# mlaaks/coherent-rtlsdr

Hardware: AMD Instinct MI355X
Metric: aligned IQ blocks/s (1024 ch x 8192) (higher is better)
Workload: dtype f32

## Files before the change

coherent-rtlsdr_amd/csrc/crsdr.hip:

```cpp
#include "../../include/crsdr.h"
#include "kernels.hpp"
#include "doa.hpp"

#include <hip/hip_runtime.h>

#include <cctype>
#include <cmath>
#include <cstdarg>
#include <cstdio>
#include <cstdlib>
#include <cstring>
#include <mutex>
#include <new>
#include <string>
#include <vector>
#include <sched.h>

using namespace crsdr;

static thread_local char g_err[512] = "";

static int fail(int code, const char *fmt, ...)
{
    va_list ap;
// ... 130 lines not shown
static int make_twiddles14(float2 **d_twA, float2 **d_twB)
{
    std::vector<float2> a(5 * 512), b(5 * 16);
    for (int j = 0; j < 5; ++j) {
        for (int t = 0; t < 512; ++t) {
            double ang = 2.0 * M_PI * (double)(t << j) / 16384.0;
            a[j * 512 + t] = make_float2((float)std::cos(ang), (float)(-std::sin(ang)));
        }
        for (int n = 0; n < 16; ++n) {
            double ang = 2.0 * M_PI * (double)(n << j) / 512.0;
            b[j * 16 + n] = make_float2((float)std::cos(ang), (float)(-std::sin(ang)));
        }
    }
    HIP_TRY(hipMalloc((void **)d_twA, sizeof(float2) * a.size()));
    HIP_TRY(hipMalloc((void **)d_twB, sizeof(float2) * b.size()));
    HIP_TRY(hipMemcpy(*d_twA, a.data(), sizeof(float2) * a.size(), hipMemcpyHostToDevice));
    HIP_TRY(hipMemcpy(*d_twB, b.data(), sizeof(float2) * b.size(), hipMemcpyHostToDevice));
    return CRSDR_OK;
}

static int make_twiddle_table(double n, size_t count, size_t step, float2 **d)
{
    std::vector<float2> h(count);
    for (size_t k = 0; k < count; ++k) {
        double a = 2.0 * M_PI * (double)(k * step) / n;
        h[k] = make_float2((float)std::cos(a), (float)(-std::sin(a)));
    }
    HIP_TRY(hipMalloc((void **)d, sizeof(float2) * count));
    HIP_TRY(hipMemcpy(*d, h.data(), sizeof(float2) * count, hipMemcpyHostToDevice));
    return CRSDR_OK;
}

constexpr int kMinLog2 = 4, kMaxLog2 = 14, kMaxLog2Plan = 22;

template <int LOG2N>
static constexpr size_t fft_lds_bytes() { return sizeof(float2) * ((size_t)1 << LOG2N) + 256; }

struct SpinSwitch {
    int value, dflt;
    long from;
    int at(long launch) const { return launch >= from ? value : dflt; }
};
static SpinSwitch spin_switch(const char *e, int dflt)
{
    const char *at = e ? strchr(e, '@') : nullptr;
    return {e ? atoi(e) : dflt, dflt, at ? atol(at + 1) : 0L};
}
struct Switches {
    char k1_variant;
    SpinSwitch qspin;
    SpinSwitch refspin;
    int k2_spin;
    bool long_q;
};
static const Switches &sw()
{
    static const Switches s = [] {
        const char *v = getenv("CRSDR_K1_VARIANT"), *lq = getenv("CRSDR_LONG_Q");
        const char c = v ? v[0] : 'a';
        return Switches{(c == 'p' || c == 'q') ? c : 'a', spin_switch(getenv("CRSDR_K1_QSPIN"), x14p::kQSpinLimit),
                        spin_switch(getenv("CRSDR_K1_REFSPIN"), kRefWaitBudget), spin_switch(getenv("CRSDR_K2_SPIN"), kFusedSpinLimit).value,
                        !lq || atoi(lq) != 0};
    }();
    return s;
}

static int device_cus()
{
    static const int cus = [] {
        int dev = 0, n = 0;
        if (hipGetDevice(&dev) != hipSuccess || hipDeviceGetAttribute(&n, hipDeviceAttributeMultiprocessorCount, dev) != hipSuccess || n < 1) n = 256;
        return n;
    }();
    return cus;
}
static char k1_pick(int rows_all, bool allow_q)
{
    char variant = sw().k1_variant;
    if (variant == 'a') variant = rows_all >= 12 * device_cus() ? 'q' : 'p';
    if (variant == 'q' && !allow_q) variant = 'p';
    return variant;
}

template <typename Kernel, typename... Args>
static hipError_t launch_lds(Kernel kern, dim3 grid, dim3 block, size_t lds, hipStream_t s, const Args &...args)
{
    const hipError_t e = hipFuncSetAttribute((const void *)kern, hipFuncAttributeMaxDynamicSharedMemorySize, (int)lds);
    if (e != hipSuccess) return e;
    hipLaunchKernelGGL(kern, grid, block, lds, s, args...);
    return hipGetLastError();
}

template <int LOG2N>
static hipError_t launch_ref_spectrum(hipStream_t s, int nblocks, const int8_t *rows, size_t block_stride, const float2 *tw,
                                      float2 *refspec, uint32_t xor80)
{
    return launch_lds(k_ref_spectrum<LOG2N>, dim3(nblocks), dim3(FftGeom<LOG2N>::THREADS), fft_lds_bytes<LOG2N>(), s, rows, block_stride, tw,
                      refspec, xor80);
}

template <int LOG2N>
static hipError_t launch_xcorr_lag(hipStream_t s, const XcorrArgs &a, int row_count, const float2 *tw)
{
    return launch_lds(k_xcorr_lag<LOG2N>, dim3(row_count, a.nblocks), dim3(FftGeom<LOG2N>::THREADS), fft_lds_bytes<LOG2N>(), s, a, tw);
}

static hipError_t launch_ref_spectrum14(hipStream_t s, int nblocks, const int8_t *rows, size_t block_stride, const float2 *twA,
                                        const float2 *twB, float2 *refspec, uint32_t xor80)
{
    return launch_lds(x14p::k_ref_spectrum14p, dim3(nblocks), dim3(x14::THREADS), x14::LDS_BYTES, s, rows, block_stride,
                      reinterpret_cast<const c2 *>(twA), reinterpret_cast<const c2 *>(twB), (float4 *)refspec, xor80);
}

static hipError_t launch_xcorr_lag14(hipStream_t s, char variant, const XcorrArgs &a, int row_count, const float2 *twA, const float2 *twB,
                                     int *waitflag, unsigned int *work, unsigned int *work_base)
{
    const int items = row_count * a.nblocks + (a.fold ? a.nblocks : 0);
    if (variant != 'q')
        return launch_lds(x14p::k_xcorr_lag14p, dim3((unsigned)items), dim3(x14::THREADS), x14::LDS_BYTES, s, a, twA, twB, row_count);
    static long launches = 0;
    const int qspin = sw().qspin.at(launches++);
    const hipError_t e = launch_lds(x14p::k_xcorr_lag14q, dim3((unsigned)std::max(1, std::min(device_cus(), (items + 1) / 2))), dim3(2 * x14p::QG),
                                    x14p::LDSQ_BYTES, s, a, twA, twB, row_count, waitflag, work, *work_base, qspin);
    if (e == hipSuccess) *work_base += (unsigned)items;
    return e;
}

template <int LOG2N, int DIR>
static hipError_t launch_op_fft(hipStream_t s, int howmany, float2 *out, const float2 *in, const float2 *tw)
{
    return launch_lds(k_op_fft<LOG2N, DIR>, dim3(howmany), dim3(FftGeom<LOG2N>::THREADS), fft_lds_bytes<LOG2N>(), s, out, in, tw);
}

#define CRSDR_DISPATCH_N1(l2, CALL)                                                     \
    [&]() -> hipError_t {                                                               \
        switch (l2) {                                                                   \
        case 1: { constexpr int LG = 1; return CALL; }                                  \
        case 2: { constexpr int LG = 2; return CALL; }                                  \
        case 3: { constexpr int LG = 3; return CALL; }                                  \
        case 4: { constexpr int LG = 4; return CALL; }                                  \
        case 5: { constexpr int LG = 5; return CALL; }                                  \
        case 6: { constexpr int LG = 6; return CALL; }                                  \
        case 7: { constexpr int LG = 7; return CALL; }                                  \
        case 8: { constexpr int LG = 8; return CALL; }                                  \
        default: return hipErrorInvalidValue;                                           \
        }                                                                               \
    }()

static int lb_grid(int nwork, bool stage_c = false)
{
    const int per_cu = stage_c ? 0 : 2;
#ifdef CRSDR_LB_EXPERIMENT
    static const int dbg_set = [] { const char *e = getenv("CRSDR_LB_DBG"); int v = e ? atoi(e) : 0; (void)hipMemcpyToSymbol(HIP_SYMBOL(lb::lb_dbg), &v, sizeof(v)); return v; }();
    (void)dbg_set;
#endif
    return per_cu > 0 ? std::max(1, std::min(nwork, per_cu * device_cus())) : nwork;
}
template <int LOG2N1, bool IS_REF>
static hipError_t launch_long_fwd_cols(hipStream_t s, int nrows_launch, const int8_t *rows, int row_begin, uint32_t xor80,
                                       const lb::LongTw &tw, float2 *Y)
{
    const int nwork = lb::ntiles(LOG2N1) * nrows_launch;
    return launch_lds(lb::k_long_fwd_cols<LOG2N1, IS_REF>, dim3((unsigned)lb_grid(nwork)), dim3(lb::THREADS), lb::LDS_BYTES, s, rows, row_begin,
                      xor80, tw, Y, nwork);
}
static hipError_t launch_long_rows_q(hipStream_t s, int n1, int nrows_launch, float2 *Y, const float2 *twA, const float2 *twB, float2 *refspec,
                                     int *waitflag, const x14p::RampArgs *ramp = nullptr, float2 *Yout = nullptr)
{
    const int items = n1 * nrows_launch;
    const int grid = std::max(1, std::min(device_cus(), (items + 1) / 2));
    const int nq = (!ramp && n1 % 8 == 0 && grid % 8 == 0) ? 8 : 1;
    static long launches = 0;
    const int qspin = sw().qspin.at(launches++);
    return launch_lds(ramp ? x14p::k_rows14_cf32q<true> : x14p::k_rows14_cf32q<false>, dim3((unsigned)grid), dim3(2 * x14p::QG), x14p::LDSQ_BYTES, s,
                      reinterpret_cast<c2 *>(Y), reinterpret_cast<const c2 *>(twA), reinterpret_cast<const c2 *>(twB), (const float4 *)refspec, n1,
// ... 323 lines not shown
    if (mem_kind == CRSDR_MEM_HOST) HIP_TRY(hipMemcpy(pm, d_p, pb, hipMemcpyDeviceToHost));
    else HIP_TRY(hipDeviceSynchronize());
    return CRSDR_OK;
}

constexpr int kStageSlots = 4;
constexpr unsigned kWaitTwoRow = 1u, kWaitTwoLine = 2u, kWaitFoldRef = 4u;
constexpr int kMaxBatch = 64;

struct crsdr_plan {
    int nrows = 0, B = 0, L = 0, log2n = 0, mode = 0, device = 0, row_begin = 1, row_count = 0, max_batch = 1;
    size_t packet_bytes = 0, matrix_off = 0, packet_stride = 0, own_packet_stride = 0;
    hipStream_t own_stream = nullptr, stream = nullptr, aux = nullptr;
    hipEvent_t ev_fork = nullptr, ev_ref[2] = {nullptr, nullptr}, ev_k1done[2] = {nullptr, nullptr};
    hipStream_t cs = nullptr;
    hipEvent_t ev_copydone[4] = {nullptr, nullptr, nullptr, nullptr};
    unsigned long copy_head = 0, copy_tail = 0;
    int *h_k1flag = nullptr;
    bool copy_pending = false;
    hipEvent_t ev_k2done[2] = {nullptr, nullptr};
    int obuf = 0;
    hipEvent_t ev_start = nullptr, ev_stop = nullptr;
    bool k1done_valid[2] = {false, false};
    bool fold_last[2] = {false, false};
    int slot = 0;
    float2 *d_tw = nullptr, *d_twA = nullptr, *d_twB = nullptr, *d_refspec[2] = {nullptr, nullptr};
    int8_t *d_rows = nullptr;
    uint8_t *d_packet_alloc = nullptr;
    int8_t *d_packet_own = nullptr, *d_packet = nullptr;
    int8_t *d_slab = nullptr;
    size_t slab_stride = 0, tail_offset = 0;
    int hdr_first = 0, hdr_count = 0;
    uint32_t *d_readcnt = nullptr;
    uint8_t *d_mask = nullptr;
    int32_t *d_lag = nullptr, *d_lag_state = nullptr;
    float *d_mag = nullptr, *d_frac = nullptr, *d_mag_state = nullptr, *d_frac_state = nullptr;
    float2 *d_phasor = nullptr, *d_phase_state[2] = {nullptr, nullptr};
    long long *d_corr = nullptr;
    int chain_slot = 0;
    int chain_armed[2] = {0, 0};
    unsigned int *d_sync = nullptr;
    unsigned int q_work_base = 0;
    bool k1_used = false;
    unsigned k1_waits = 0;
    uint8_t *d_state = nullptr, *d_state_snap = nullptr;
    size_t state_bytes = 0;
    bool q_disabled = false;
    static constexpr int kSnaps = 8;
    struct Snap { unsigned long idx; int phase_cur; } snaps[kSnaps] = {};
    int snap_head = 0, snap_cnt = 0;
    unsigned long submit_idx = 0;
    unsigned long copy_idx[4] = {0, 0, 0, 0};
    bool fused_k2 = true;
    bool fold = true;
    unsigned int *d_refflag = nullptr, refgen = 0;
    int phase_cur = 0;
    int last_nblocks = 0;
    bool longblock = false;
    int log2n1 = 0;
    float2 *d_wc = nullptr, *d_wf = nullptr, *d_tw1 = nullptr, *d_Y = nullptr, *d_Yref = nullptr;
    lb::LongPartial *d_part = nullptr;
    int long_chunk = 1 << 30;
    bool frac_apply = false, frac_override_on = false;
    float frac_gain = 1.0f;
    float *d_frac_override = nullptr;
    uint32_t *d_k2tab = nullptr;
    bool frac_generic = false;
    float2 *d_Z = nullptr;
    float4 *d_rowspec = nullptr;
    uint32_t *h_readcnt = nullptr;
    uint8_t *h_mask = nullptr;
    hipEvent_t ev_stage[kStageSlots] = {};
    bool stage_valid[kStageSlots] = {};
    int stage_slot = 0;
    bool submitted = false;
    int prof_slots = 0;
    uint32_t prof_mask = 0;
    long prof_count = 0;
    std::vector<hipEvent_t> prof_ev;
    std::vector<unsigned char> prof_has;
};

constexpr int kProfKernels = 4;

static hipEvent_t *prof_pair(crsdr_plan *p, int which)
{
    if (!p->prof_slots || !(p->prof_mask & (1u << which))) return nullptr;
    const int slot = (int)(p->prof_count % p->prof_slots);
    p->prof_has[(size_t)slot * kProfKernels + which] = 1;
    return &p->prof_ev[((size_t)slot * kProfKernels + which) * 2];
}

static int plan_init_state(crsdr_plan *p)
{
    const size_t n = (size_t)p->nrows, T = (size_t)p->max_batch;
    std::vector<float2> ph(n, make_float2(1.0f, 0.0f));
    ph[0] = make_float2(0.0f, 0.0f);
    for (int i = 0; i < 2; ++i) HIP_TRY(hipMemcpy(p->d_phase_state[i], ph.data(), sizeof(float2) * n, hipMemcpyHostToDevice));
    for (size_t t = 0; t < T; ++t) HIP_TRY(hipMemcpy(p->d_phasor + t * n, ph.data(), sizeof(float2) * n, hipMemcpyHostToDevice));
    HIP_TRY(hipMemset(p->d_lag, 0, sizeof(int32_t) * n * T * 2));
    HIP_TRY(hipMemset(p->d_mag, 0, sizeof(float) * n * T * 2));
    HIP_TRY(hipMemset(p->d_frac, 0, sizeof(float) * n * T * 2));
    HIP_TRY(hipMemset(p->d_lag_state, 0, sizeof(int32_t) * n));
    HIP_TRY(hipMemset(p->d_mag_state, 0, sizeof(float) * n));
    HIP_TRY(hipMemset(p->d_frac_state, 0, sizeof(float) * n));
    HIP_TRY(hipMemset(p->d_corr, 0xFF, sizeof(long long) * 4 * n * T));
    p->chain_armed[0] = p->chain_armed[1] = (int)T;
// ... 38 lines not shown
{
    HIP_TRY(hipSetDevice(p->device));
    HIP_TRY(hipStreamCreateWithFlags(&p->own_stream, hipStreamNonBlocking));
    HIP_TRY(hipStreamCreateWithFlags(&p->aux, hipStreamNonBlocking));
    HIP_TRY(hipStreamCreateWithFlags(&p->cs, hipStreamNonBlocking));
    for (auto &e : p->ev_copydone) HIP_TRY(hipEventCreateWithFlags(&e, hipEventDisableTiming));
    HIP_TRY(hipHostMalloc((void **)&p->h_k1flag, 4 * sizeof(int), hipHostMallocDefault));
    memset(p->h_k1flag, 0, 4 * sizeof(int));
    p->stream = p->own_stream;
    hipEvent_t *evs[] = {&p->ev_fork, &p->ev_ref[0], &p->ev_ref[1], &p->ev_k1done[0], &p->ev_k1done[1], &p->ev_k2done[0], &p->ev_k2done[1]};
    for (auto e : evs) HIP_TRY(hipEventCreateWithFlags(e, hipEventDisableTiming));
    for (int i = 0; i < kStageSlots; ++i) HIP_TRY(hipEventCreateWithFlags(&p->ev_stage[i], hipEventDisableTiming));
    HIP_TRY(hipEventCreate(&p->ev_start));
    HIP_TRY(hipEventCreate(&p->ev_stop));
    { int rc = make_twiddles(p->longblock ? lb::N2 : p->B, &p->d_tw); if (rc) return rc; }
    if (p->log2n == 14 || p->longblock) { int rc = make_twiddles14(&p->d_twA, &p->d_twB); if (rc) return rc; }
    if (p->longblock) {
        const size_t Bz = (size_t)p->B, n1 = Bz >> lb::LOG2N2;
        int rc;
        if ((rc = make_twiddle_table((double)Bz, Bz >> lb::FBITS, (size_t)1 << lb::FBITS, &p->d_wc))) return rc;
        if ((rc = make_twiddle_table((double)Bz, (size_t)1 << lb::FBITS, 1, &p->d_wf))) return rc;
        if ((rc = make_twiddle_table((double)n1, n1, 1, &p->d_tw1))) return rc;
        HIP_TRY(hipMalloc((void **)&p->d_Y, sizeof(float2) * Bz * (size_t)p->row_count));
        HIP_TRY(hipMalloc((void **)&p->d_Yref, sizeof(float2) * Bz));
        {
            const char *e = getenv("CRSDR_LONG_CHUNK_MB");
            const long mb = e ? atol(e) : 400;
            if (mb > 0) p->long_chunk = (int)std::max<size_t>(1, ((size_t)mb << 20) / (sizeof(float2) * Bz));
        }
        HIP_TRY(hipMalloc((void **)&p->d_part, sizeof(lb::LongPartial) * (size_t)lb::ntiles(p->log2n1) * (size_t)p->row_count));
    }
    const size_t n = (size_t)p->nrows, T = (size_t)p->max_batch;
    const size_t rowbytes = n * (size_t)p->B;
    for (int i = 0; i < 2; ++i) HIP_TRY(hipMalloc((void **)&p->d_refspec[i], sizeof(float2) * (size_t)p->B * T));
    HIP_TRY(hipMalloc((void **)&p->d_rows, rowbytes * T));
    const size_t pad = (256 - (p->matrix_off % 256)) % 256;
    p->own_packet_stride = (p->packet_bytes + 255) / 256 * 256;
    p->packet_stride = p->own_packet_stride;
    HIP_TRY(hipMalloc((void **)&p->d_packet_alloc, pad + p->own_packet_stride * T + 256));
    HIP_TRY(hipMemset(p->d_packet_alloc, 0, pad + p->own_packet_stride * T + 256));
    p->d_packet_own = reinterpret_cast<int8_t *>(p->d_packet_alloc + pad);
    p->d_packet = p->d_packet_own;
    HIP_TRY(hipMalloc((void **)&p->d_readcnt, sizeof(uint32_t) * n * T));
    HIP_TRY(hipMalloc((void **)&p->d_mask, n));
    HIP_TRY(hipMalloc((void **)&p->d_lag, sizeof(int32_t) * n * T * 2));
    HIP_TRY(hipMalloc((void **)&p->d_mag, sizeof(float) * n * T * 2));
    HIP_TRY(hipMalloc((void **)&p->d_frac, sizeof(float) * n * T * 2));
    HIP_TRY(hipMalloc((void **)&p->d_phasor, sizeof(float2) * n * T));
    HIP_TRY(hipMalloc((void **)&p->d_corr, sizeof(long long) * 4 * n * T));
    HIP_TRY(hipMalloc((void **)&p->d_sync, 64));
    HIP_TRY(hipMemset(p->d_sync, 0, 64));
    HIP_TRY(hipMalloc((void **)&p->d_refflag, sizeof(unsigned int) * T));
    HIP_TRY(hipMemset(p->d_refflag, 0, sizeof(unsigned int) * T));
    { const char *e = getenv("CRSDR_K1_FOLD"); if (e) p->fold = atoi(e) != 0; }
    { const char *e = getenv("CRSDR_K2_FUSED"); if (e) p->fused_k2 = atoi(e) != 0; }
    { const char *e = getenv("CRSDR_FRAC_GENERIC"); if (e) p->frac_generic = atoi(e) != 0; }
    {
        const size_t n8 = (n + 1) / 2 * 2;
        p->state_bytes = n8 * (3 * 4 + 2 * 8);
        HIP_TRY(hipMalloc((void **)&p->d_state, p->state_bytes));
        HIP_TRY(hipMalloc((void **)&p->d_state_snap, p->state_bytes * crsdr_plan::kSnaps));
        p->d_phase_state[0] = reinterpret_cast<float2 *>(p->d_state);
        p->d_phase_state[1] = p->d_phase_state[0] + n8;
        p->d_lag_state = reinterpret_cast<int32_t *>(p->d_phase_state[1] + n8);
        p->d_mag_state = reinterpret_cast<float *>(p->d_lag_state + n8);
        p->d_frac_state = p->d_mag_state + n8;
    }
    HIP_TRY(hipHostMalloc((void **)&p->h_readcnt, sizeof(uint32_t) * n * T * kStageSlots, hipHostMallocDefault));
    HIP_TRY(hipHostMalloc((void **)&p->h_mask, n * kStageSlots, hipHostMallocDefault));
    if (p->longblock || p->log2n == 14) { int rc = make_k2tab(p); if (rc) return rc; }
    HIP_TRY(hipMalloc((void **)&p->d_frac_override, sizeof(float) * (size_t)p->nrows));
    HIP_TRY(hipMemset(p->d_frac_override, 0, sizeof(float) * (size_t)p->nrows));
    return plan_init_state(p);
}

static void plan_free(crsdr_plan *p)
{
    if (!p) return;
    (void)hipSetDevice(p->device);
    if (p->own_stream) (void)hipStreamSynchronize(p->own_stream);
    if (p->aux) (void)hipStreamSynchronize(p->aux);
    if (p->cs) { (void)hipStreamSynchronize(p->cs); (void)hipStreamDestroy(p->cs); }
    for (auto e : p->ev_copydone) if (e) (void)hipEventDestroy(e);
    void *bufs[] = {p->d_Z, p->d_rowspec, p->d_frac_override, p->d_k2tab, p->d_wc, p->d_wf, p->d_tw1, p->d_Y, p->d_Yref, p->d_part, p->d_tw, p->d_twA, p->d_twB, p->d_refspec[0], p->d_refspec[1], p->d_rows, p->d_packet_alloc, p->d_readcnt,
                    p->d_mask, p->d_lag, p->d_mag, p->d_frac, p->d_phasor, p->d_corr, p->d_sync, p->d_state, p->d_state_snap, p->d_refflag};
    for (void *b : bufs) if (b) (void)hipFree(b);
    if (p->h_k1flag) (void)hipHostFree(p->h_k1flag);
    if (p->h_readcnt) (void)hipHostFree(p->h_readcnt);
    if (p->h_mask) (void)hipHostFree(p->h_mask);
    hipEvent_t evs[] = {p->ev_fork, p->ev_ref[0], p->ev_ref[1], p->ev_k1done[0], p->ev_k1done[1], p->ev_k2done[0], p->ev_k2done[1], p->ev_start, p->ev_stop};
    for (hipEvent_t e : evs) if (e) (void)hipEventDestroy(e);
    for (int i = 0; i < kStageSlots; ++i) if (p->ev_stage[i]) (void)hipEventDestroy(p->ev_stage[i]);
    for (hipEvent_t e : p->prof_ev) if (e) (void)hipEventDestroy(e);
    if (p->own_stream) (void)hipStreamDestroy(p->own_stream);
    if (p->aux) (void)hipStreamDestroy(p->aux);
    delete p;
}

extern "C" int crsdr_plan_create(crsdr_plan **plan, const crsdr_plan_desc *desc)
{
    if (!plan || !desc) return fail(CRSDR_EINVAL, "plan_create: NULL argument");
    *plan = nullptr;
    const int l2 = ilog2_exact(desc->blocksize);
    if (desc->nrows < 2) return fail(CRSDR_EINVAL, "plan_create: nrows = %d (need the ref row and >= 1 signal row)", desc->nrows);
    if (l2 < kMinLog2 || l2 > kMaxLog2Plan)
        return fail(CRSDR_EINVAL, "plan_create: blocksize = %d unsupported (power of two in [16, 4194304])", desc->blocksize);
    if (desc->mode != CRSDR_MODE_FAITHFUL && desc->mode != CRSDR_MODE_DIGITAL)
// ... 145 lines not shown
                return fail(CRSDR_EINVAL, "plan_set_frac_apply: frac_override[%d] = %g (need |D| <= 64 samples; larger delays belong in the integer lag)", r, (double)frac_override[r]);
    HIP_TRY(hipSetDevice(p->device));
    if (frac_override) {
        int rc = crsdr_plan_sync(p);
        if (rc) return rc;
        HIP_TRY(hipMemcpy(p->d_frac_override, frac_override, sizeof(float) * (size_t)p->nrows, hipMemcpyHostToDevice));
    }
    if (!p->longblock) {
        p->frac_apply = true; p->frac_gain = gain; p->frac_override_on = frac_override != nullptr;
        return CRSDR_OK;
    }
    if (!p->d_rowspec) HIP_TRY(hipMalloc((void **)&p->d_rowspec, sizeof(float4) * 8192 * (size_t)p->row_count));
    if (enable == 2 && p->d_Z) {
        int rc = crsdr_plan_sync(p);
        if (rc) return rc;
        (void)hipFree(p->d_Z);
        p->d_Z = nullptr;
    }
    if (enable == 1 && !p->d_Z && hipMalloc((void **)&p->d_Z, sizeof(float2) * (size_t)p->B * (size_t)p->row_count) != hipSuccess) {
        p->d_Z = nullptr;
        (void)hipGetLastError();
    }
    p->frac_apply = true; p->frac_gain = gain; p->frac_override_on = frac_override != nullptr;
    return CRSDR_OK;
}

static hipError_t take_snapshot(crsdr_plan *p, hipStream_t s)
{
    if (p->snap_cnt == crsdr_plan::kSnaps) return hipSuccess;
    if (p->snap_cnt && p->snaps[(p->snap_head + p->snap_cnt - 1) % crsdr_plan::kSnaps].idx == p->submit_idx) return hipSuccess;
    const int pos = (p->snap_head + p->snap_cnt) % crsdr_plan::kSnaps;
    const hipError_t e = hipMemcpyAsync(p->d_state_snap + (size_t)pos * p->state_bytes, p->d_state, p->state_bytes, hipMemcpyDeviceToDevice, s);
    if (e != hipSuccess) return e;
    p->snaps[pos].idx = p->submit_idx;
    p->snaps[pos].phase_cur = p->phase_cur;
    p->snap_cnt++;
    return hipSuccess;
}
static void retire_snapshots(crsdr_plan *p, unsigned long k)
{
    while (p->snap_cnt >= 2 && p->snaps[(p->snap_head + 1) % crsdr_plan::kSnaps].idx <= k + 1) { p->snap_head = (p->snap_head + 1) % crsdr_plan::kSnaps; p->snap_cnt--; }
    if (p->snap_cnt == 1 && p->snaps[p->snap_head].idx <= k && p->submit_idx == k + 1) p->snap_cnt = 0;
}

struct Batch {
    int nblocks;
    const int8_t *d_in;
    size_t d_stride;
    bool input_ready;
    uint32_t xor80;
    const uint32_t *d_readcnt;
    const uint8_t *d_mask;
    bool any_lag;
    int32_t *o_lag;
    float *o_mag, *o_frac;
    AlignArgs aa;
    bool vec16;
    int chunks;
    bool fused;
    bool kept_fwd;
    bool corr_zeroed;
};

static int stage_inputs(crsdr_plan *p, Batch &b, const void *rows, int mem_kind, size_t block_stride, const uint32_t *readcnt,
                        const uint8_t *lag_mask, uint32_t flags)
{
    hipStream_t S = p->stream;
    const size_t B = (size_t)p->B, n = (size_t)p->nrows, T = (size_t)b.nblocks;
    b.d_in = (const int8_t *)rows;
    b.d_stride = block_stride;
    b.input_ready = (flags & CRSDR_INPUT_READY) && mem_kind == CRSDR_MEM_DEVICE;
    b.xor80 = (flags & CRSDR_OFFSET_BINARY) ? 0x80808080u : 0u;
    if (mem_kind == CRSDR_MEM_HOST) {
        for (size_t t = 0; t < T; ++t) {
            const int8_t *src = (const int8_t *)rows + t * block_stride;
            int8_t *dst = p->d_rows + t * n * B;
            HIP_TRY(hipMemcpyAsync(dst, src, B, hipMemcpyHostToDevice, S));
            HIP_TRY(hipMemcpyAsync(dst + B * (size_t)p->row_begin, src + B * (size_t)p->row_begin, B * (size_t)p->row_count,
                                   hipMemcpyHostToDevice, S));
        }
        b.d_in = p->d_rows;
        b.d_stride = n * B;
    }
    b.any_lag = !(flags & CRSDR_NO_LAG);
    if (readcnt || lag_mask) {
        const int ss = p->stage_slot;
        p->stage_slot = (ss + 1) % kStageSlots;
        if (p->stage_valid[ss]) HIP_TRY(hipEventSynchronize(p->ev_stage[ss]));
        if (readcnt) {
            uint32_t *h = p->h_readcnt + (size_t)ss * n * (size_t)p->max_batch;
            memcpy(h, readcnt, sizeof(uint32_t) * n * T);
            HIP_TRY(hipMemcpyAsync(p->d_readcnt, h, sizeof(uint32_t) * n * T, hipMemcpyHostToDevice, S));
            b.d_readcnt = p->d_readcnt;
        }
        if (lag_mask) {
            uint8_t *h = p->h_mask + (size_t)ss * n;
            memcpy(h, lag_mask, n);
            bool any = false;
            for (int r = p->row_begin; r < p->row_begin + p->row_count; ++r) any |= (h[r] != 0);
            b.any_lag = b.any_lag && any;
            HIP_TRY(hipMemcpyAsync(p->d_mask, h, n, hipMemcpyHostToDevice, S));
            b.d_mask = p->d_mask;
        }
        HIP_TRY(hipEventRecord(p->ev_stage[ss], S));
        p->stage_valid[ss] = true;
    }
    if (p->copy_pending) {
        hipEvent_t newest = p->ev_copydone[(p->copy_tail - 1) % 4];
        HIP_TRY(hipStreamWaitEvent(S, newest, 0));
        p->copy_pending = false;
    }
    if (p->prof_slots) {
        const int ps = (int)(p->prof_count % p->prof_slots);
        for (int k = 0; k < kProfKernels; ++k) p->prof_has[(size_t)ps * kProfKernels + k] = 0;
        if (p->prof_mask & (1u << 31)) HIP_TRY(hipEventRecord(p->ev_start, S));
    }
    return CRSDR_OK;
}

static void setup_outputs(crsdr_plan *p, Batch &b, uint32_t seq, uint32_t flags)
{
// ... 58 lines not shown

static bool two_line(const crsdr_plan *p, int cnt)
{
    const char kv = sw().k1_variant;
    return sw().long_q && (kv == 'a' || kv == 'q') && !p->q_disabled && ((long)1 << p->log2n1) * cnt >= 1024;
}

static int k1_long(crsdr_plan *p, Batch &b)
{
    hipStream_t S = p->stream;
    const lb::LongTw tw{p->d_wc, p->d_wf, p->d_tw1, p->d_tw, (uint32_t)(p->B - 1)};
    const int n1 = 1 << p->log2n1, l1 = p->log2n1;
    const int slot = (p->slot ^= 1);
    int rc = run_k0(p, b, slot, [&](hipStream_t A) -> int {
        HIP_TRY(CRSDR_DISPATCH_N1(l1, (launch_long_fwd_cols<LG, true>(A, 1, b.d_in, 0, b.xor80, tw, p->d_Yref))));
        HIP_TRY(launch_long_rows<true>(A, n1, 1, p->d_Yref, p->d_twA, p->d_twB, p->d_refspec[slot]));
        return CRSDR_OK;
    });
    if (rc) return rc;
    hipEvent_t *pe1 = prof_pair(p, CRSDR_KERNEL_XCORR_LAG);
    if (pe1) HIP_TRY(hipEventRecord(pe1[0], S));
    b.kept_fwd = p->d_Z && p->frac_apply && b.aa.digital;
    for (int r0 = 0; r0 < p->row_count; r0 += p->long_chunk) b.kept_fwd = b.kept_fwd && two_line(p, std::min(p->long_chunk, p->row_count - r0));
    for (int r0 = 0; r0 < p->row_count; r0 += p->long_chunk) {
        const int cnt = std::min(p->long_chunk, p->row_count - r0);
        float2 *Yc = p->d_Y + (size_t)r0 * (size_t)p->B;
        float2 *Zc = b.kept_fwd ? p->d_Z + (size_t)r0 * (size_t)p->B : Yc;
        HIP_TRY(CRSDR_DISPATCH_N1(l1, (launch_long_fwd_cols<LG, false>(S, cnt, b.d_in, p->row_begin + r0, b.xor80, tw, Yc))));
        if (two_line(p, cnt)) {
            HIP_TRY(take_snapshot(p, S));
            HIP_TRY(launch_long_rows_q(S, n1, cnt, Yc, p->d_twA, p->d_twB, p->d_refspec[slot], reinterpret_cast<int *>(p->d_sync + 2), nullptr,
                                       Zc != Yc ? Zc : nullptr));
            p->k1_used = true;
            p->k1_waits |= kWaitTwoLine;
        } else
            HIP_TRY(launch_long_rows<false>(S, n1, cnt, Yc, p->d_twA, p->d_twB, p->d_refspec[slot]));
        HIP_TRY(CRSDR_DISPATCH_N1(l1, (launch_long_inv_cols<LG>(S, cnt, Zc, tw, p->d_part + (size_t)r0 * lb::ntiles(l1), nullptr))));
    }
    HIP_TRY(hipEventRecord(p->ev_k1done[slot], S));
    p->k1done_valid[slot] = true;
    b.corr_zeroed = b.aa.refnoise && !b.fused && b.chunks > 1 && b.nblocks == 1;
    hipLaunchKernelGGL(lb::k_long_finalize, dim3(p->row_count), dim3(256), 0, S, b.kept_fwd ? p->d_Z : p->d_Y, p->d_part, tw, n1, lb::ntiles(l1),
                       xcorr_args(p, b, slot), b.corr_zeroed ? p->d_corr : nullptr);
    HIP_TRY(hipGetLastError());
    if (pe1) HIP_TRY(hipEventRecord(pe1[1], S));
    return CRSDR_OK;
}

static int k1_short(crsdr_plan *p, Batch &b)
{
    hipStream_t S = p->stream;
    const int slot = (p->slot ^= 1);
    const char variant = p->log2n == 14 ? k1_pick(p->row_count * b.nblocks, !p->q_disabled) : 0;
    const bool fold = p->fold && p->log2n == 14 && !p->q_disabled && variant == 'p';
    if (!fold) {
        int rc = run_k0(p, b, slot, [&](hipStream_t A) -> int {
            if (p->log2n == 14) HIP_TRY(launch_ref_spectrum14(A, b.nblocks, b.d_in, b.d_stride, p->d_twA, p->d_twB, p->d_refspec[slot], b.xor80));
            else HIP_TRY(CRSDR_DISPATCH_LOG2(p->log2n, (launch_ref_spectrum<LG>(A, b.nblocks, b.d_in, b.d_stride, p->d_tw, p->d_refspec[slot], b.xor80))));
            return CRSDR_OK;
        });
        if (rc) return rc;
    }
    XcorrArgs xa = xcorr_args(p, b, slot);
    if (fold) {
        static long folded = 0;
        xa.fold = 1; xa.refspec_w = p->d_refspec[slot]; xa.refflag = p->d_refflag; xa.refgen = ++p->refgen;
        xa.errflag = reinterpret_cast<int *>(p->d_sync + 2);
        xa.refspin = sw().refspin.at(folded++);
    }
    hipEvent_t *pe1 = prof_pair(p, CRSDR_KERNEL_XCORR_LAG);
    if (pe1) HIP_TRY(hipEventRecord(pe1[0], S));
    if (p->log2n == 14) {
        const bool q = variant == 'q';
        if (q || fold) HIP_TRY(take_snapshot(p, S));
        HIP_TRY(launch_xcorr_lag14(S, variant, xa, p->row_count, p->d_twA, p->d_twB, reinterpret_cast<int *>(p->d_sync + 2), p->d_sync + 3, &p->q_work_base));
        p->k1_used |= q || fold;
        p->k1_waits |= (q ? kWaitTwoRow : 0u) | (fold ? kWaitFoldRef : 0u);
    } else
        HIP_TRY(CRSDR_DISPATCH_LOG2(p->log2n, (launch_xcorr_lag<LG>(S, xa, p->row_count, p->d_tw))));
    if (pe1) HIP_TRY(hipEventRecord(pe1[1], S));
    if (!fold) {
        HIP_TRY(hipEventRecord(p->ev_k1done[slot], S));
        p->k1done_valid[slot] = true;
    } else
        p->fold_last[slot] = true;
    return CRSDR_OK;
}

static int frac_pass(crsdr_plan *p, const Batch &b);

static int phase_fused(crsdr_plan *p, const Batch &b)
{
    hipStream_t S = p->stream;
    const size_t n = (size_t)p->nrows;
    const int nblocks = b.nblocks;
    const int cs = p->chain_slot;
    unsigned long long *chain = reinterpret_cast<unsigned long long *>(p->d_corr);
    unsigned long long *chainv = chain + 2 * n * (size_t)p->max_batch;
    const bool rn = b.aa.refnoise;
    FusedSync fs{p->d_sync, p->d_sync + 1, chain + cs, rn ? chain + (cs ^ 1) : nullptr, chainv + cs, rn ? chainv + (cs ^ 1) : nullptr,
                 p->row_count, sw().k2_spin};
    hipEvent_t *pe = prof_pair(p, CRSDR_KERNEL_ALIGN_QUANT);
    if (pe) HIP_TRY(hipEventRecord(pe[0], S));
    if (rn) {
        if (nblocks > 1 && p->chain_armed[cs] < nblocks) {
            HIP_TRY(hipMemsetAsync(p->d_corr, 0xFF, sizeof(long long) * 4 * n * (size_t)nblocks, S));
            p->chain_armed[0] = p->chain_armed[1] = nblocks;
// ... 546 lines not shown
```

coherent-rtlsdr_amd/csrc/xcorr14q.hpp:

```cpp
#pragma once
#include "xcorr14p.hpp"

namespace crsdr {
namespace x14p {

constexpr int QG = 256;
constexpr int QSCR_BYTES = 64 + 4 * 2 * 64 * 4;
constexpr int LDSQ_BYTES = LDS_ELEMS * 8 + 2 * QSCR_BYTES + 64;
constexpr int kQSpinLimit = 1 << 18;
#ifndef Q_PRIO
#define Q_PRIO 3
#endif
#ifndef Q_ACQ_SLEEP
#define Q_ACQ_SLEEP 2
#endif

struct QSync {
    int owner;
    int relcnt;
    int bar[2];
    int err;
    int next[2];
    int spin_limit;
    int arrive[2];
};
static_assert(sizeof(QSync) <= 64, "QSync must fit the 64 bytes reserved behind the scratch");

#ifdef CRSDR_QDEBUG
__device__ unsigned long long *dbg__ = nullptr;
#define QDBG_T0 const unsigned long long t0__ = __builtin_readcyclecounter();
#define QDBG_ADD(slot) if (dbg__ && blockIdx.x == 0 && (threadIdx.x & 63) == 0) atomicAdd(dbg__ + (slot), (unsigned long long)(__builtin_readcyclecounter() - t0__));
#else
#define QDBG_T0
#define QDBG_ADD(slot)
#endif
__device__ __forceinline__ void q_barrier(QSync *s, int g, int &gen, int site = 0)
{
    QDBG_T0
    __builtin_amdgcn_fence(__ATOMIC_RELEASE, "workgroup");
    if ((threadIdx.x & 63) == 0) __hip_atomic_fetch_add(&s->bar[g], 1, __ATOMIC_RELAXED, __HIP_MEMORY_SCOPE_WORKGROUP);
    gen += QG / 64;
    int spins = 0;
    while (__hip_atomic_load(&s->bar[g], __ATOMIC_RELAXED, __HIP_MEMORY_SCOPE_WORKGROUP) < gen) {
        if (++spins > s->spin_limit || __hip_atomic_load(&s->err, __ATOMIC_RELAXED, __HIP_MEMORY_SCOPE_WORKGROUP)) {
            __hip_atomic_store(&s->err, 1, __ATOMIC_RELAXED, __HIP_MEMORY_SCOPE_WORKGROUP);
            break;
        }
    }
    __builtin_amdgcn_fence(__ATOMIC_ACQUIRE, "workgroup");
    QDBG_ADD(1)
    QDBG_ADD(3 + site)
}

__device__ __forceinline__ void q_acquire(QSync *s, int tag)
{
    QDBG_T0
    int spins = 0;
    for (;;) {
        int old = tag;
        if ((threadIdx.x & 63) == 0) {
            int expected = 0;
// ... 161 lines not shown
    case 29: asm volatile("v_mov_b32 %0, %1" : "=v"(r) : "v"(m0[29])); break;
    case 30: asm volatile("v_mov_b32 %0, %1" : "=v"(r) : "v"(m0[30])); break;
    case 31: asm volatile("v_mov_b32 %0, %1" : "=v"(r) : "v"(m0[31])); break;
    case 32: asm volatile("v_mov_b32 %0, %1" : "=v"(r) : "v"(m1[0])); break;
    case 33: asm volatile("v_mov_b32 %0, %1" : "=v"(r) : "v"(m1[1])); break;
    case 34: asm volatile("v_mov_b32 %0, %1" : "=v"(r) : "v"(m1[2])); break;
    case 35: asm volatile("v_mov_b32 %0, %1" : "=v"(r) : "v"(m1[3])); break;
    case 36: asm volatile("v_mov_b32 %0, %1" : "=v"(r) : "v"(m1[4])); break;
    case 37: asm volatile("v_mov_b32 %0, %1" : "=v"(r) : "v"(m1[5])); break;
    case 38: asm volatile("v_mov_b32 %0, %1" : "=v"(r) : "v"(m1[6])); break;
    case 39: asm volatile("v_mov_b32 %0, %1" : "=v"(r) : "v"(m1[7])); break;
    case 40: asm volatile("v_mov_b32 %0, %1" : "=v"(r) : "v"(m1[8])); break;
    case 41: asm volatile("v_mov_b32 %0, %1" : "=v"(r) : "v"(m1[9])); break;
    case 42: asm volatile("v_mov_b32 %0, %1" : "=v"(r) : "v"(m1[10])); break;
    case 43: asm volatile("v_mov_b32 %0, %1" : "=v"(r) : "v"(m1[11])); break;
    case 44: asm volatile("v_mov_b32 %0, %1" : "=v"(r) : "v"(m1[12])); break;
    case 45: asm volatile("v_mov_b32 %0, %1" : "=v"(r) : "v"(m1[13])); break;
    case 46: asm volatile("v_mov_b32 %0, %1" : "=v"(r) : "v"(m1[14])); break;
    case 47: asm volatile("v_mov_b32 %0, %1" : "=v"(r) : "v"(m1[15])); break;
    case 48: asm volatile("v_mov_b32 %0, %1" : "=v"(r) : "v"(m1[16])); break;
    case 49: asm volatile("v_mov_b32 %0, %1" : "=v"(r) : "v"(m1[17])); break;
    case 50: asm volatile("v_mov_b32 %0, %1" : "=v"(r) : "v"(m1[18])); break;
    case 51: asm volatile("v_mov_b32 %0, %1" : "=v"(r) : "v"(m1[19])); break;
    case 52: asm volatile("v_mov_b32 %0, %1" : "=v"(r) : "v"(m1[20])); break;
    case 53: asm volatile("v_mov_b32 %0, %1" : "=v"(r) : "v"(m1[21])); break;
    case 54: asm volatile("v_mov_b32 %0, %1" : "=v"(r) : "v"(m1[22])); break;
    case 55: asm volatile("v_mov_b32 %0, %1" : "=v"(r) : "v"(m1[23])); break;
    case 56: asm volatile("v_mov_b32 %0, %1" : "=v"(r) : "v"(m1[24])); break;
    case 57: asm volatile("v_mov_b32 %0, %1" : "=v"(r) : "v"(m1[25])); break;
    case 58: asm volatile("v_mov_b32 %0, %1" : "=v"(r) : "v"(m1[26])); break;
    case 59: asm volatile("v_mov_b32 %0, %1" : "=v"(r) : "v"(m1[27])); break;
    case 60: asm volatile("v_mov_b32 %0, %1" : "=v"(r) : "v"(m1[28])); break;
    case 61: asm volatile("v_mov_b32 %0, %1" : "=v"(r) : "v"(m1[29])); break;
    case 62: asm volatile("v_mov_b32 %0, %1" : "=v"(r) : "v"(m1[30])); break;
    case 63: asm volatile("v_mov_b32 %0, %1" : "=v"(r) : "v"(m1[31])); break;
    default: break;
    }
    return r;
}

__global__ __launch_bounds__(2 * QG, 1) void k_xcorr_lag14q(XcorrArgs a, const float2 *__restrict__ twA_, const float2 *__restrict__ twB_,
                                                           int row_count, int *__restrict__ errflag, unsigned int *__restrict__ work,
                                                           unsigned int work_base, int spin_limit)
{
    extern __shared__ __attribute__((aligned(16))) unsigned char smem[];
    const c2 *twA = reinterpret_cast<const c2 *>(twA_), *twB = reinterpret_cast<const c2 *>(twB_);
    c2 *A = reinterpret_cast<c2 *>(smem);
    float4 *A4 = reinterpret_cast<float4 *>(smem);
    const int g = threadIdx.x >> 8, tid = threadIdx.x & (QG - 1);
    float *red = reinterpret_cast<float *>(smem + (size_t)LDS_ELEMS * 8 + QSCR_BYTES * g);
    int *redi = reinterpret_cast<int *>(red);
    float *edge = red + 16;
    QSync *sy = reinterpret_cast<QSync *>(smem + (size_t)LDS_ELEMS * 8 + 2 * QSCR_BYTES);
    if (threadIdx.x == 0) { sy->owner = 0; sy->relcnt = 0; sy->bar[0] = 0; sy->bar[1] = 0; sy->err = 0; sy->next[0] = 0; sy->next[1] = 0; sy->spin_limit = spin_limit; sy->arrive[0] = 0; sy->arrive[1] = 0; }
    __syncthreads();
    int gen = 0;
#ifdef CRSDR_QDEBUG
    const unsigned long long tk0__ = __builtin_readcyclecounter();
#endif
    const int nitems = row_count * a.nblocks;
    int item = g * (int)gridDim.x + (int)blockIdx.x;
    for (int k = 0;; ++k) {
        int vt0 = tid, vt1 = tid + QG;
        asm volatile("" : "+v"(vt0), "+v"(vt1));
        if ((unsigned)item >= (unsigned)nitems) break;
        const int item_u = __builtin_amdgcn_readfirstlane(item);
        const int t = item_u / row_count, row = a.row_begin + item_u % row_count;
        if (xcorr_skip(a, row, t, tid)) {
            q_barrier(sy, g, gen, 5);
            if (tid == 0) sy->next[g] = 2 * (int)gridDim.x + (int)(atomicAdd(work, 1u) - work_base);
            q_barrier(sy, g, gen, 5);
            item = sy->next[g];
            continue;
        }
        const int8_t *src = a.rows + (size_t)t * a.block_stride + (size_t)row * N;
        const float4 *__restrict__ refspec4 = reinterpret_cast<const float4 *>(a.refspec) + (size_t)t * (N / 2);
        c2 wB[32];
        {
            c2 v[32], v2[32];
            q_p0_compute(v, src, twA, a.xor80, vt0);
            q_p0_compute(v2, src, twA, a.xor80, vt1);
            tw_load(wB, twB, TWB_STRIDE, tid & 15);
            q_acquire(sy, 2 * k + g + 1);
            __builtin_amdgcn_s_setprio(Q_PRIO);
            q_p0_store(A, v, vt0);
            q_p0_store(A, v2, vt1);
        }
        float4 ra[8], rb[8];
        q_refspec_load(ra, refspec4, vt0, 0);
        q_barrier(sy, g, gen, 0);
        int drawn = 0;
        if (tid == 0) drawn = 2 * (int)gridDim.x + (int)(atomicAdd(work, 1u) - work_base);
        pass1_forward<true>(A, wB, vt0);
        pass1_forward<true>(A, wB, vt1);
        wave_lds_sync();
        q_refspec_load(rb, refspec4, vt0, 1);
        q_junction_half<true>(A4, ra, vt0, 0);
        q_refspec_load(ra, refspec4, vt1, 0);
        q_junction_half<true>(A4, rb, vt0, 1);
        q_refspec_load(rb, refspec4, vt1, 1);
        q_junction_half<true>(A4, ra, vt1, 0);
        q_junction_half<true>(A4, rb, vt1, 1);
        wave_lds_sync();
        pass1_inverse<true>(A, wB, vt0);
        pass1_inverse<true>(A, wB, vt1);
        if (tid == 0) sy->next[g] = drawn;
        q_barrier(sy, g, gen, 1);
        float m0[32], m1[32];
        {
            c2 v[32], v2[32];
            q_p0i_load(v, A, vt0);
            q_p0i_load(v2, A, vt1);
            q_release(sy);
            __builtin_amdgcn_s_setprio(0);
            int vb0 = tid, vb1 = tid + QG;
            asm volatile("" : "+v"(vb0), "+v"(vb1));
            q_p0i_compute(m0, v, twA, vb0);
            q_p0i_compute(m1, v2, twA, vb1);
        }
        float tm = fmaxf(m0[0], m1[0]);
#pragma unroll
        for (int i = 1; i < 32; ++i) tm = fmaxf(tm, fmaxf(m0[i], m1[i]));
        const int lane = tid & 63, wv = tid >> 6;
        const float wm = __int_as_float(__builtin_amdgcn_readlane(__float_as_int(q_wave_max63(tm)), 63));
        int bi = 0x7fffffff;
        if (tm == wm) {
#pragma unroll
            for (int i = 31; i >= 0; --i) {
                bi = (m1[i] == wm) ? i * 512 + vt1 : bi;
                bi = (m0[i] == wm) ? i * 512 + vt0 : bi;
            }
        }
        const int wbi = q_wave_min(bi);
        if (lane == 0 || lane == 63) {
            float4 *e4 = reinterpret_cast<float4 *>(edge + (wv * 2 + (lane ? 1 : 0)) * 64);
// ... 195 lines not shown
```

Measured before the change: 23090.

## Fold reference-spectrum computation into the persistent q-variant xcorr kernel

Extends the fold path (computing the reference spectrum inside the xcorr kernel, signalled through per-block flags) from the 'p' variant to the persistent 'q' variant. The first nblocks workgroups compute a reference row before entering the work loop, and consumers wait on the refflag once per new time block. By default the fold is used only when the previous K2 has finished, checked with an event query. This removes a separate ref-spectrum launch and its serialization, but adds spin-waiting on flags and a grid large enough to cover nblocks.

After: 23200 (median of 6 runs). About the same (+0.5%).

```diff
diff --git a/coherent-rtlsdr_amd/csrc/crsdr.hip b/coherent-rtlsdr_amd/csrc/crsdr.hip
--- a/coherent-rtlsdr_amd/csrc/crsdr.hip
+++ b/coherent-rtlsdr_amd/csrc/crsdr.hip
@@ -206,15 +206,17 @@
     SpinSwitch refspin;
     int k2_spin;
     bool long_q;
+    int k1_fold;
 };
 static const Switches &sw()
 {
     static const Switches s = [] {
-        const char *v = getenv("CRSDR_K1_VARIANT"), *lq = getenv("CRSDR_LONG_Q");
+        const char *v = getenv("CRSDR_K1_VARIANT"), *lq = getenv("CRSDR_LONG_Q"), *kf = getenv("CRSDR_K1_FOLD");
         const char c = v ? v[0] : 'a';
+        const int fold = kf ? atoi(kf) : 1;
         return Switches{(c == 'p' || c == 'q') ? c : 'a', spin_switch(getenv("CRSDR_K1_QSPIN"), x14p::kQSpinLimit),
                         spin_switch(getenv("CRSDR_K1_REFSPIN"), kRefWaitBudget), spin_switch(getenv("CRSDR_K2_SPIN"), kFusedSpinLimit).value,
-                        !lq || atoi(lq) != 0};
+                        !lq || atoi(lq) != 0, (fold >= 0 && fold <= 3) ? fold : 1};
     }();
     return s;
 }
@@ -269,12 +271,13 @@
 static hipError_t launch_xcorr_lag14(hipStream_t s, char variant, const XcorrArgs &a, int row_count, const float2 *twA, const float2 *twB,
                                      int *waitflag, unsigned int *work, unsigned int *work_base)
 {
-    const int items = row_count * a.nblocks + (a.fold ? a.nblocks : 0);
+    const int items = row_count * a.nblocks;
     if (variant != 'q')
-        return launch_lds(x14p::k_xcorr_lag14p, dim3((unsigned)items), dim3(x14::THREADS), x14::LDS_BYTES, s, a, twA, twB, row_count);
+        return launch_lds(x14p::k_xcorr_lag14p, dim3((unsigned)(items + (a.fold ? a.nblocks : 0))), dim3(x14::THREADS), x14::LDS_BYTES, s, a, twA, twB, row_count);
     static long launches = 0;
     const int qspin = sw().qspin.at(launches++);
-    const hipError_t e = launch_lds(x14p::k_xcorr_lag14q, dim3((unsigned)std::max(1, std::min(device_cus(), (items + 1) / 2))), dim3(2 * x14p::QG),
+    const int grid = std::max(std::max(1, std::min(device_cus(), (items + 1) / 2)), a.fold ? a.nblocks : 0);
+    const hipError_t e = launch_lds(x14p::k_xcorr_lag14q, dim3((unsigned)grid), dim3(2 * x14p::QG),
                                     x14p::LDSQ_BYTES, s, a, twA, twB, row_count, waitflag, work, *work_base, qspin);
     if (e == hipSuccess) *work_base += (unsigned)items;
     return e;
@@ -704,7 +707,6 @@
     unsigned long submit_idx = 0;
     unsigned long copy_idx[4] = {0, 0, 0, 0};
     bool fused_k2 = true;
-    bool fold = true;
     unsigned int *d_refflag = nullptr, refgen = 0;
     int phase_cur = 0;
     int last_nblocks = 0;
@@ -849,7 +851,6 @@
     HIP_TRY(hipMemset(p->d_sync, 0, 64));
     HIP_TRY(hipMalloc((void **)&p->d_refflag, sizeof(unsigned int) * T));
     HIP_TRY(hipMemset(p->d_refflag, 0, sizeof(unsigned int) * T));
-    { const char *e = getenv("CRSDR_K1_FOLD"); if (e) p->fold = atoi(e) != 0; }
     { const char *e = getenv("CRSDR_K2_FUSED"); if (e) p->fused_k2 = atoi(e) != 0; }
     { const char *e = getenv("CRSDR_FRAC_GENERIC"); if (e) p->frac_generic = atoi(e) != 0; }
     {
@@ -1101,6 +1102,7 @@
     const uint32_t *d_readcnt;
     const uint8_t *d_mask;
     bool any_lag;
+    bool plan_idle;
     int32_t *o_lag;
     float *o_mag, *o_frac;
     AlignArgs aa;
@@ -1116,6 +1118,12 @@
 {
     hipStream_t S = p->stream;
     const size_t B = (size_t)p->B, n = (size_t)p->nrows, T = (size_t)b.nblocks;
+    b.plan_idle = true;
+    if (p->submitted && p->log2n == 14 && sw().k1_fold == 1 && !p->q_disabled) {
+        const hipError_t q = hipEventQuery(p->ev_k2done[p->obuf]);
+        if (q == hipErrorNotReady) { b.plan_idle = false; (void)hipGetLastError(); }
+        else HIP_TRY(q);
+    }
     b.d_in = (const int8_t *)rows;
     b.d_stride = block_stride;
     b.input_ready = (flags & CRSDR_INPUT_READY) && mem_kind == CRSDR_MEM_DEVICE;
@@ -1280,7 +1288,8 @@
     hipStream_t S = p->stream;
     const int slot = (p->slot ^= 1);
     const char variant = p->log2n == 14 ? k1_pick(p->row_count * b.nblocks, !p->q_disabled) : 0;
-    const bool fold = p->fold && p->log2n == 14 && !p->q_disabled && variant == 'p';
+    const int fold_rule = sw().k1_fold;
+    const bool fold = fold_rule && p->log2n == 14 && !p->q_disabled && (variant == 'p' || (variant == 'q' && (fold_rule == 2 || (fold_rule == 1 && b.plan_idle))));
     if (!fold) {
         int rc = run_k0(p, b, slot, [&](hipStream_t A) -> int {
             if (p->log2n == 14) HIP_TRY(launch_ref_spectrum14(A, b.nblocks, b.d_in, b.d_stride, p->d_twA, p->d_twB, p->d_refspec[slot], b.xor80));
diff --git a/coherent-rtlsdr_amd/csrc/xcorr14q.hpp b/coherent-rtlsdr_amd/csrc/xcorr14q.hpp
--- a/coherent-rtlsdr_amd/csrc/xcorr14q.hpp
+++ b/coherent-rtlsdr_amd/csrc/xcorr14q.hpp
@@ -7,6 +7,7 @@
 constexpr int QG = 256;
 constexpr int QSCR_BYTES = 64 + 4 * 2 * 64 * 4;
 constexpr int LDSQ_BYTES = LDS_ELEMS * 8 + 2 * QSCR_BYTES + 64;
+static_assert(LDSQ_BYTES <= 160 * 1024, "one workgroup per CU: the image, the scratch and the sync words fit a CU's LDS");
 constexpr int kQSpinLimit = 1 << 18;
 #ifndef Q_PRIO
 #define Q_PRIO 3
@@ -274,6 +275,13 @@
     int *redi = reinterpret_cast<int *>(red);
     float *edge = red + 16;
     QSync *sy = reinterpret_cast<QSync *>(smem + (size_t)LDS_ELEMS * 8 + 2 * QSCR_BYTES);
+    if (a.fold && (int)blockIdx.x < a.nblocks) {
+        const int rb = (int)blockIdx.x;
+        ref_spectrum_row14<true>(smem, a.rows + (size_t)rb * a.block_stride, twA, twB, reinterpret_cast<float4 *>(a.refspec_w) + (size_t)rb * (N / 2), a.xor80);
+        asm volatile("s_waitcnt vmcnt(0)" ::: "memory");
+        __syncthreads();
+        if (threadIdx.x == 0) __hip_atomic_store(a.refflag + rb, a.refgen, __ATOMIC_RELAXED, __HIP_MEMORY_SCOPE_AGENT);
+    }
     if (threadIdx.x == 0) { sy->owner = 0; sy->relcnt = 0; sy->bar[0] = 0; sy->bar[1] = 0; sy->err = 0; sy->next[0] = 0; sy->next[1] = 0; sy->spin_limit = spin_limit; sy->arrive[0] = 0; sy->arrive[1] = 0; }
     __syncthreads();
     int gen = 0;
@@ -281,6 +289,7 @@
     const unsigned long long tk0__ = __builtin_readcyclecounter();
 #endif
     const int nitems = row_count * a.nblocks;
+    int ref_seen = a.fold ? -1 : 0x7fffffff;
     int item = g * (int)gridDim.x + (int)blockIdx.x;
     for (int k = 0;; ++k) {
         int vt0 = tid, vt1 = tid + QG;
@@ -297,12 +306,21 @@
         }
         const int8_t *src = a.rows + (size_t)t * a.block_stride + (size_t)row * N;
         const float4 *__restrict__ refspec4 = reinterpret_cast<const float4 *>(a.refspec) + (size_t)t * (N / 2);
+        const bool ref_look = t > ref_seen;
+        unsigned int ref_early = 0u;
+        if (ref_look && tid < 64) ref_early = word_peek(a.refflag + t);
         c2 wB[32];
         {
             c2 v[32], v2[32];
             q_p0_compute(v, src, twA, a.xor80, vt0);
             q_p0_compute(v2, src, twA, a.xor80, vt1);
             tw_load(wB, twB, TWB_STRIDE, tid & 15);
+            if (ref_look) {
+                if (tid < 64 && (a.refspin < 0 || !wait_word(a.refflag + t, a.refgen, ref_early, a.refspin)))
+                    __hip_atomic_store(&sy->err, 1, __ATOMIC_RELAXED, __HIP_MEMORY_SCOPE_WORKGROUP);
+                q_barrier(sy, g, gen, 5);
+                ref_seen = t;
+            }
             q_acquire(sy, 2 * k + g + 1);
             __builtin_amdgcn_s_setprio(Q_PRIO);
             q_p0_store(A, v, vt0);
```
